# Eclectic-Sheep/sheeprl

Hardware: NVIDIA H100
Metric: Dreamer-V3 train-steps/sec (S, bs16 seq64 horizon15, 64x64x3 obs) (higher is better)
Workload: dtype f32

## Files before the change

sheeprl_b200/csrc/gemm_tc.cu:

```cuda
#include <cuda.h>
#include <cudaTypedefs.h>

#include <mutex>
#include <unordered_map>

#include "common.cuh"

namespace {

constexpr int BM = 128, BK = 32;
constexpr int NTHREADS = 384;
constexpr int NSPLIT_THREADS = 96;
constexpr int NCONS_WARPS = 8;
constexpr int PRODUCER_REGS = 56, CONSUMER_REGS = 224;
template <int PASSES, bool PRESPLIT> __host__ __device__ constexpr int b_buffers() { return PRESPLIT ? (PASSES == 3 ? 2 : 1) : 3; }
template <int BN, int PASSES, bool PRESPLIT> constexpr int stages_for() {
  return (227 * 1024 - 1024 - 256) / ((BM + b_buffers<PASSES, PRESPLIT>() * BN) * BK * (int)sizeof(float));
}

__device__ __forceinline__ uint32_t smem_u32(const void* p) { return (uint32_t)__cvta_generic_to_shared(p); }

__device__ __forceinline__ void mbar_init(uint64_t* bar, uint32_t count) {
  asm volatile("mbarrier.init.shared::cta.b64 [%0], %1;" ::"r"(smem_u32(bar)), "r"(count) : "memory");
}
__device__ __forceinline__ void mbar_expect_tx(uint64_t* bar, uint32_t bytes) {
  asm volatile("mbarrier.arrive.expect_tx.shared::cta.b64 _, [%0], %1;" ::"r"(smem_u32(bar)), "r"(bytes) : "memory");
}
__device__ __forceinline__ void mbar_arrive(uint64_t* bar) {
  asm volatile("mbarrier.arrive.shared::cta.b64 _, [%0];" ::"r"(smem_u32(bar)) : "memory");
}
__device__ __forceinline__ bool mbar_try_wait(uint64_t* bar, uint32_t parity) {
// ... 52 lines not shown
__device__ __forceinline__ void wgmma_tf32(float (&d)[64], const uint32_t (&a)[4], uint64_t desc_b, int scale_d) {
  asm volatile(
      "{\n\t.reg .pred p;\n\tsetp.ne.b32 p, %69, 0;\n\twgmma.mma_async.sync.aligned.m64n128k8.f32.tf32.tf32 {%0, %1, %2, %3, %4, %5, %6, %7, %8, %9, %10, %11, %12, %13, %14, %15, %16, %17, %18, %19, %20, %21, %22, %23, %24, %25, %26, %27, %28, %29, %30, %31, %32, %33, %34, %35, %36, %37, %38, %39, %40, %41, %42, %43, %44, %45, %46, %47, %48, %49, %50, %51, %52, %53, %54, %55, %56, %57, %58, %59, %60, %61, %62, %63}, {%64, %65, %66, %67}, %68, p, 1, 1;\n\t}"
      : "+f"(d[0]), "+f"(d[1]), "+f"(d[2]), "+f"(d[3]), "+f"(d[4]), "+f"(d[5]), "+f"(d[6]), "+f"(d[7]), "+f"(d[8]), "+f"(d[9]), "+f"(d[10]), "+f"(d[11]), "+f"(d[12]), "+f"(d[13]), "+f"(d[14]), "+f"(d[15]), "+f"(d[16]), "+f"(d[17]), "+f"(d[18]), "+f"(d[19]), "+f"(d[20]), "+f"(d[21]), "+f"(d[22]), "+f"(d[23]), "+f"(d[24]), "+f"(d[25]), "+f"(d[26]), "+f"(d[27]), "+f"(d[28]), "+f"(d[29]), "+f"(d[30]), "+f"(d[31]), "+f"(d[32]), "+f"(d[33]), "+f"(d[34]), "+f"(d[35]), "+f"(d[36]), "+f"(d[37]), "+f"(d[38]), "+f"(d[39]), "+f"(d[40]), "+f"(d[41]), "+f"(d[42]), "+f"(d[43]), "+f"(d[44]), "+f"(d[45]), "+f"(d[46]), "+f"(d[47]), "+f"(d[48]), "+f"(d[49]), "+f"(d[50]), "+f"(d[51]), "+f"(d[52]), "+f"(d[53]), "+f"(d[54]), "+f"(d[55]), "+f"(d[56]), "+f"(d[57]), "+f"(d[58]), "+f"(d[59]), "+f"(d[60]), "+f"(d[61]), "+f"(d[62]), "+f"(d[63])
      : "r"(a[0]), "r"(a[1]), "r"(a[2]), "r"(a[3]), "l"(desc_b), "r"(scale_d));
}
__device__ __forceinline__ void wgmma_fence() { asm volatile("wgmma.fence.sync.aligned;" ::: "memory"); }
__device__ __forceinline__ void wgmma_commit() { asm volatile("wgmma.commit_group.sync.aligned;" ::: "memory"); }
__device__ __forceinline__ void wgmma_wait_all() { asm volatile("wgmma.wait_group.sync.aligned 0;" ::: "memory"); }
template <int N>
__device__ __forceinline__ void fence_regs(float (&r)[N]) {
#pragma unroll
  for (int i = 0; i < N; ++i) asm volatile("" : "+f"(r[i])::"memory");
}
template <int N, int W>
__device__ __forceinline__ void fence_regs(uint32_t (&r)[N][W]) {
#pragma unroll
  for (int i = 0; i < N; ++i)
#pragma unroll
    for (int j = 0; j < W; ++j) asm volatile("" : "+r"(r[i][j])::"memory");
}

__device__ __forceinline__ uint64_t make_desc(uint32_t smem_addr) {
  uint64_t d = 0;
  d |= (uint64_t)((smem_addr & 0x3FFFF) >> 4);
  d |= (uint64_t)1 << 16;
  d |= (uint64_t)(1024 >> 4) << 32;
  d |= (uint64_t)1 << 62;
  return d;
}

__device__ __forceinline__ uint32_t kmajor_off(int r, int k) {
  return (uint32_t)(r * 128 + ((((k >> 2) ^ r) & 7) << 4) + (k & 3) * 4);
}
__device__ __forceinline__ uint32_t mnmajor_off(int r, int k) {
  return (uint32_t)((r >> 5) * 4096 + k * 128 + (((((r & 31) >> 2) ^ k) & 7) << 4) + (r & 3) * 4);
}

template <int BN, int PASSES, bool PRESPLIT>
struct Smem;
template <int BN, int PASSES>
struct Smem<BN, PASSES, false> {
  static constexpr int STAGES = stages_for<BN, PASSES, false>();
  float a[STAGES][BM * BK];
  float b[STAGES][BN * BK];
  float b_hi[STAGES][BN * BK];
  float b_lo[STAGES][BN * BK];
  uint64_t full[STAGES], split[STAGES], empty[STAGES];
};
template <int BN, int PASSES>
struct Smem<BN, PASSES, true> {
  static constexpr int STAGES = stages_for<BN, PASSES, true>();
  float a[STAGES][BM * BK];
  float b_hi[STAGES][BN * BK];
  float b_lo[PASSES == 3 ? STAGES : 1][PASSES == 3 ? BN * BK : 256];
  uint64_t full[STAGES], empty[STAGES];
};

constexpr int CH = 4;

constexpr int MODE_GEMM = 0, MODE_DOWN = 1, MODE_UP = 2;
constexpr int MODE_UP4 = 3;
constexpr int GROUP_M = 16;
struct TileGeo {
  int mode;
  int h, w, NB;
  int bw, bh, bn;
  int tiles_x, tiles_y;
  int chunks;
  int Cout;
  int ksplits;
  float* part;
  int mpad, ldw;
  int force_part;
  int passes;
  int a_mn, b_mn;
  int mtiles;
  int ntiles;
  int wg;
};

template <int BN, int PASSES, bool PRESPLIT>
__global__ void __launch_bounds__(NTHREADS, 1)
gemm_tc_kernel(const __grid_constant__ CUtensorMap mapA, const __grid_constant__ CUtensorMap mapB,
               const __grid_constant__ CUtensorMap mapBlo, float* __restrict__ C, const float* __restrict__ bias, int M,
               int N, int K, int ldc, int accumulate, const TileGeo geo) {
  using S = Smem<BN, PASSES, PRESPLIT>;
  constexpr int STAGES = S::STAGES;
  extern __shared__ __align__(1024) unsigned char smem_raw[];
  S& s = *reinterpret_cast<S*>(smem_raw + ((1024u - (smem_u32(smem_raw) & 1023u)) & 1023u));
  const int warp = threadIdx.x >> 5, lane = threadIdx.x & 31;
  const int mtiles = geo.mtiles * geo.ntiles, tstride = gridDim.y;
  auto tile_mn = [&](int id, int& tm, int& tn) {
    if (geo.ntiles == 1) { tm = id; tn = 0; return; }
    const int per = GROUP_M * geo.ntiles, grp = id / per, first = grp * GROUP_M;
    const int gsz = min(GROUP_M, geo.mtiles - first), r = id - grp * per;
    tn = r / gsz;
    tm = first + (r - tn * gsz);
  };
  int kb_base = 0, nkb = (K + BK - 1) / BK;
  if (geo.mode == MODE_GEMM && geo.ksplits > 1) {
    const int per = (nkb + geo.ksplits - 1) / geo.ksplits;
    kb_base = (int)blockIdx.z * per;
    nkb = min(per, nkb - kb_base);
  }
  const int py = (int)blockIdx.z >> 1, px = (int)blockIdx.z & 1;
  auto tile_origin = [&](int id, int& tx0, int& ty0, int& tn0) {
    tx0 = (id % geo.tiles_x) * geo.bw;
    ty0 = ((id / geo.tiles_x) % geo.tiles_y) * geo.bh;
    tn0 = (id / (geo.tiles_x * geo.tiles_y)) * geo.bn;
  };

  if (threadIdx.x == 0) {
    for (int i = 0; i < STAGES; ++i) {
      mbar_init(&s.full[i], 1);
      if constexpr (!PRESPLIT) mbar_init(&s.split[i], NSPLIT_THREADS / 32);
      mbar_init(&s.empty[i], NCONS_WARPS);
    }
    asm volatile("fence.mbarrier_init.release.cluster;" ::: "memory");
  }
  __syncthreads();

  if (warp < 4) {
    asm volatile("setmaxnreg.dec.sync.aligned.u32 %0;" ::"n"(PRODUCER_REGS));
    if (warp == 0) {
      const bool leader = elect_one();
      constexpr uint32_t STAGE_TX = (uint32_t)((BM + (PRESPLIT ? b_buffers<PASSES, true>() : 1) * BN) * BK * sizeof(float));
      auto load_b_kmajor = [&](int st, int k, int n) {
        if constexpr (PRESPLIT) {
          tma_load_2d(s.b_hi[st], &mapB, &s.full[st], k, n);
          if (PASSES == 3) tma_load_2d(s.b_lo[st], &mapBlo, &s.full[st], k, n);
        } else {
          tma_load_2d(s.b[st], &mapB, &s.full[st], k, n);
        }
      };
      int it = 0;
      for (int tile = blockIdx.y; tile < mtiles; tile += tstride) {
        int tm, tn;
        tile_mn(tile, tm, tn);
        const int m0 = tm * BM, n0 = tn * BN;
        int tx0 = 0, ty0 = 0, tn0 = 0;
        if (geo.mode != MODE_GEMM) tile_origin(tm, tx0, ty0, tn0);
        for (int kb = 0; kb < nkb; ++kb, ++it) {
          const int st = it % STAGES;
          if (it >= STAGES) mbar_wait(&s.empty[st], ((it / STAGES) - 1) & 1);
          if (leader) {
            mbar_expect_tx(&s.full[st], STAGE_TX);
            if (geo.mode == MODE_GEMM) {
              const int k0 = (kb_base + kb) * BK;
              if (geo.wg) {
                const int x0 = k0 % geo.w, y0 = (k0 / geo.w) % geo.h, i0 = k0 / (geo.w * geo.h);
                for (int j = 0; j < BM / 32; ++j) {
                  const int r0 = m0 + 32 * j, tap = r0 / geo.Cout, ch = r0 - tap * geo.Cout;
                  tma_load_4d(s.a[st] + j * 1024, &mapA, &s.full[st], ch, 2 * x0 - 1 + (tap & 3), 2 * y0 - 1 + (tap >> 2), i0);
                }
              } else if (!geo.a_mn) tma_load_2d(s.a[st], &mapA, &s.full[st], k0, m0);
              else
                for (int j = 0; j < BM / 32; ++j) tma_load_2d(s.a[st] + j * 1024, &mapA, &s.full[st], m0 + 32 * j, k0);
              if (PRESPLIT || !geo.b_mn) load_b_kmajor(st, k0, n0);
              else if constexpr (!PRESPLIT)
                for (int j = 0; j < BN / 32; ++j) tma_load_2d(s.b[st] + j * 1024, &mapB, &s.full[st], n0 + 32 * j, k0);
            } else {
              const int tap = kb / geo.chunks, ch = (kb - tap * geo.chunks) * BK;
              int x, y;
              if (geo.mode == MODE_DOWN)     { x = 2 * tx0 - 1 + (tap & 3); y = 2 * ty0 - 1 + (tap >> 2); }
              else if (geo.mode == MODE_UP4) { x = tx0 + (tap % 3) - 1;     y = ty0 + (tap / 3) - 1; }
              else                           { x = tx0 + px - (tap & 1);    y = ty0 + py - (tap >> 1); }
              tma_load_4d(s.a[st], &mapA, &s.full[st], ch, x, y, tn0);
              load_b_kmajor(st, kb * BK, n0 + (geo.mode == MODE_UP ? (int)blockIdx.z * geo.Cout : 0));
            }
          }
          __syncwarp();
        }
      }
    } else if constexpr (!PRESPLIT) {
      const int t = threadIdx.x - 32;
      int ntl = 0;
      for (int tile = blockIdx.y; tile < mtiles; tile += tstride) ++ntl;
      const int total_kb = ntl * nkb;
      const bool b_mn = geo.b_mn != 0;
      for (int kb = 0; kb < total_kb; ++kb) {
        const int st = kb % STAGES;
        mbar_wait(&s.full[st], (kb / STAGES) & 1);
        const char* raw = reinterpret_cast<const char*>(s.b[st]);
// ... 17 lines not shown
          h.x = __uint_as_float(__float_as_uint(v.x) & 0xffffe000u);
          h.y = __uint_as_float(__float_as_uint(v.y) & 0xffffe000u);
          h.z = __uint_as_float(__float_as_uint(v.z) & 0xffffe000u);
          h.w = __uint_as_float(__float_as_uint(v.w) & 0xffffe000u);
          const uint32_t o = kmajor_off(n, 4 * kc);
          *reinterpret_cast<float4*>(bh + o) = h;
          if (PASSES == 3) *reinterpret_cast<float4*>(bl + o) = make_float4(v.x - h.x, v.y - h.y, v.z - h.z, v.w - h.w);
        }
        asm volatile("fence.proxy.async.shared::cta;" ::: "memory");
        __syncwarp();
        if (lane == 0) mbar_arrive(&s.split[st]);
      }
    }
  } else {
    asm volatile("setmaxnreg.inc.sync.aligned.u32 %0;" ::"n"(CONSUMER_REGS));
    constexpr int NACC = BN / 2;
    const int cw = (warp >> 2) - 1, wq = warp & 3, g = lane >> 2, tq = lane & 3;
    const int r0 = cw * 64 + wq * 16 + g;
    const bool a_mn_tile = geo.a_mn != 0;
    const uint64_t dbh_base = make_desc(smem_u32(s.b_hi[0])), dbl_base = make_desc(smem_u32(s.b_lo[0]));
    constexpr uint64_t STAGE_STEP = (uint64_t)(BN * BK * sizeof(float)) >> 4;
    int it = 0;
    for (int tile = blockIdx.y; tile < mtiles; tile += tstride) {
      int tm, tn;
      tile_mn(tile, tm, tn);
      const int m0 = tm * BM, n0 = tn * BN;
      int tx0 = 0, ty0 = 0, tn0 = 0;
      if (geo.mode != MODE_GEMM) tile_origin(tm, tx0, ty0, tn0);
      float acc[NACC], cacc[NACC];
#pragma unroll
      for (int j = 0; j < NACC; ++j) { acc[j] = 0.f; cacc[j] = 0.f; }
      for (int kb = 0; kb < nkb; ++kb, ++it) {
        const int st = it % STAGES;
        const uint32_t ph = (it / STAGES) & 1;
        mbar_wait(&s.full[st], ph);
        if constexpr (!PRESPLIT) mbar_wait(&s.split[st], ph);
        const char* araw = reinterpret_cast<const char*>(s.a[st]);
        uint32_t ahi[4][4], alo[4][4];
#pragma unroll
        for (int ks = 0; ks < 4; ++ks)
#pragma unroll
          for (int e = 0; e < 4; ++e) {
            const int r = r0 + 8 * (e & 1), k = 8 * ks + tq + 4 * (e >> 1);
            const uint32_t x = *reinterpret_cast<const uint32_t*>(araw + (a_mn_tile ? mnmajor_off(r, k) : kmajor_off(r, k)));
            ahi[ks][e] = x & 0xffffe000u;
            if (PASSES == 3) alo[ks][e] = __float_as_uint(__uint_as_float(x) - __uint_as_float(x & 0xffffe000u));
          }
        const bool chunk_start = (kb % CH) == 0;
        const uint64_t dbh0 = dbh_base + (uint64_t)st * STAGE_STEP, dbl0 = dbl_base + (uint64_t)st * STAGE_STEP;
        fence_regs(cacc);
        fence_regs(ahi);
        if (PASSES == 3) fence_regs(alo);
        wgmma_fence();
#pragma unroll
        for (int ks = 0; ks < 4; ++ks) {
          const uint64_t ob = (uint64_t)ks * 2;
          const int keep = !(chunk_start && ks == 0);
          if (PASSES == 3) {
            wgmma_tf32(cacc, ahi[ks], dbl0 + ob, keep);
            wgmma_tf32(cacc, alo[ks], dbh0 + ob, 1);
            wgmma_tf32(cacc, ahi[ks], dbh0 + ob, 1);
          } else {
            wgmma_tf32(cacc, ahi[ks], dbh0 + ob, keep);
          }
        }
        wgmma_commit();
        wgmma_wait_all();
        fence_regs(cacc);
        fence_regs(ahi);
        if (PASSES == 3) fence_regs(alo);
        __syncwarp();
        if (lane == 0) mbar_arrive(&s.empty[st]);
        if ((kb % CH) == CH - 1 || kb == nkb - 1) {
#pragma unroll
          for (int j = 0; j < NACC; ++j) acc[j] += cacc[j];
        }
      }
#pragma unroll
      for (int hh = 0; hh < 2; ++hh) {
        const int r = r0 + 8 * hh;
        const int row = m0 + r;
        bool row_ok = row < M;
        size_t row_off = (size_t)row * ldc;
        int wi = 0, hi = 0, ni = 0;
        if (geo.mode != MODE_GEMM) {
          wi = r % geo.bw; hi = (r / geo.bw) % geo.bh; ni = r / (geo.bw * geo.bh);
          const int n = tn0 + ni, y = ty0 + hi, x = tx0 + wi;
          row_ok = n < geo.NB;
          if (geo.mode == MODE_DOWN) row_off = (((size_t)n * geo.h + y) * geo.w + x) * (size_t)ldc;
          else row_off = (((size_t)n * (2 * geo.h) + (2 * y + py)) * (2 * geo.w) + (2 * x + px)) * (size_t)ldc;
        }
        if (geo.mode == MODE_UP4) {
          if (!row_ok) continue;
          const size_t n = (size_t)(tn0 + ni);
          const int y = ty0 + hi, x = tx0 + wi;
#pragma unroll
          for (int j = 0; j < NACC / 4; ++j) {
            const int c = 8 * j + 2 * tq, p = c >> 5, ch = c & 31;
            float* dst = C + ((n * (2 * geo.h) + (2 * y + (p >> 1))) * (2 * geo.w) + (2 * x + (p & 1))) * (size_t)32 + ch;
            float2 o = make_float2(acc[4 * j + 2 * hh], acc[4 * j + 2 * hh + 1]);
            if (bias) { o.x += bias[ch]; o.y += bias[ch + 1]; }
            *reinterpret_cast<float2*>(dst) = o;
          }
          continue;
        }
        if (geo.mode == MODE_GEMM && (geo.ksplits > 1 || geo.force_part)) {
          float* prow = geo.part + ((size_t)blockIdx.z * geo.mpad + (size_t)row) * geo.ldw + n0;
#pragma unroll
          for (int j = 0; j < NACC / 4; ++j)
            *reinterpret_cast<float2*>(prow + 8 * j + 2 * tq) = make_float2(acc[4 * j + 2 * hh], acc[4 * j + 2 * hh + 1]);
          continue;
        }
        if (!row_ok) continue;
        float* crow = C + row_off;
#pragma unroll
        for (int j = 0; j < NACC / 4; ++j) {
          const int cb = n0 + 8 * j + 2 * tq;
          float v0 = acc[4 * j + 2 * hh], v1 = acc[4 * j + 2 * hh + 1];
          if (cb + 1 < N && ((reinterpret_cast<uintptr_t>(crow + cb) & 7) == 0)) {
            if (bias) { v0 += bias[cb]; v1 += bias[cb + 1]; }
            if (accumulate) { const float2 q = *reinterpret_cast<const float2*>(crow + cb); v0 += q.x; v1 += q.y; }
            *reinterpret_cast<float2*>(crow + cb) = make_float2(v0, v1);
          } else {
            if (cb < N) crow[cb] = v0 + (bias ? bias[cb] : 0.f) + (accumulate ? crow[cb] : 0.f);
            if (cb + 1 < N) crow[cb + 1] = v1 + (bias ? bias[cb + 1] : 0.f) + (accumulate ? crow[cb + 1] : 0.f);
          }
        }
      }
    }
  }
}

struct MapKey {
// ... 155 lines not shown
  store_split(P, L, idx, W[((long long)cs * Cb + cb) * 16 + tap]);
}
__global__ void conv_pack_up_kernel(const float* __restrict__ W, float* __restrict__ P, float* __restrict__ L, int Cs,
                                    int Cb) {
  const long long idx = (long long)blockIdx.x * blockDim.x + threadIdx.x;
  if (idx >= (long long)Cs * Cb * 16) return;
  const int cs = (int)(idx % Cs);
  const int t = (int)((idx / Cs) % 4);
  const int cb = (int)((idx / ((long long)Cs * 4)) % Cb);
  const int par = (int)(idx / ((long long)Cs * 4 * Cb));
  const int py = par >> 1, px = par & 1;
  const int ky = (1 - py) + 2 * (t >> 1), kx = (1 - px) + 2 * (t & 1);
  store_split(P, L, idx, W[((long long)cs * Cb + cb) * 16 + ky * 4 + kx]);
}

__global__ void conv_pack_up4_kernel(const float* __restrict__ W, float* __restrict__ P, float* __restrict__ L, int Cs,
                                     int Cb) {
  const long long idx = (long long)blockIdx.x * blockDim.x + threadIdx.x;
  if (idx >= 36LL * Cs * Cb) return;
  const int cs = (int)(idx % Cs);
  const int shift = (int)((idx / Cs) % 9);
  const int cb = (int)((idx / (9LL * Cs)) % Cb);
  const int par = (int)(idx / (9LL * Cs * Cb));
  const int py = par >> 1, px = par & 1, dy = shift / 3 - 1, dx = shift % 3 - 1;
  const int j = py - dy, i = px - dx;
  float v = 0.f;
  if (j >= 0 && j <= 1 && i >= 0 && i <= 1) v = W[((long long)cs * Cb + cb) * 16 + ((1 - py) + 2 * j) * 4 + (1 - px) + 2 * i];
  store_split(P, L, idx, v);
}
static bool conv_up_merged(int Cb) { return Cb == 32; }

int g_passes = 3;

struct SplitWs {
  float* part = nullptr;
  size_t floats = 0;
};
SplitWs g_split[16];
std::mutex g_split_mu;

int split_workspace(size_t need_floats, cudaStream_t st, float** part) {
  int dev = 0;
// ... 37 lines not shown
  if (n + 4 <= N && ((reinterpret_cast<uintptr_t>(c) & 15) == 0)) {
    float4 r = acc;
    if (bias) { r.x += bias[n]; r.y += bias[n + 1]; r.z += bias[n + 2]; r.w += bias[n + 3]; }
    if (accumulate) { const float4 q = *reinterpret_cast<const float4*>(c); r.x += q.x; r.y += q.y; r.z += q.z; r.w += q.w; }
    *reinterpret_cast<float4*>(c) = r;
  } else {
    for (int j = 0; j < 4 && n + j < N; ++j) {
      float r = o[j];
      if (bias) r += bias[n + j];
      if (accumulate) r += c[j];
      c[j] = r;
    }
  }
}

#define LAUNCH_GEMM_TC(BN_, PASSES_, PRE_, grid_, st_, ...)                                                          \
  do {                                                                                                               \
    static_assert(sizeof(Smem<BN_, PASSES_, PRE_>) + 1024 <= 227 * 1024, "operand stages exceed shared memory");     \
    const size_t smem__ = sizeof(Smem<BN_, PASSES_, PRE_>) + 1024;                                                   \
    RL_CUDA(cudaFuncSetAttribute(gemm_tc_kernel<BN_, PASSES_, PRE_>, cudaFuncAttributeMaxDynamicSharedMemorySize,     \
                                 (int)smem__));                                                                      \
    gemm_tc_kernel<BN_, PASSES_, PRE_><<<grid_, NTHREADS, smem__, st_>>>(__VA_ARGS__);                                \
  } while (0)
#define DISPATCH_GEMM_TC_PRE(BN_val, passes_val, PRE_, grid_, st_, ...)                        \
  do {                                                                                          \
    if ((BN_val) == 64) {                                                                       \
      if ((passes_val) == 3) LAUNCH_GEMM_TC(64, 3, PRE_, grid_, st_, __VA_ARGS__);              \
      else LAUNCH_GEMM_TC(64, 1, PRE_, grid_, st_, __VA_ARGS__);                                \
    } else {                                                                                    \
      if ((passes_val) == 3) LAUNCH_GEMM_TC(128, 3, PRE_, grid_, st_, __VA_ARGS__);             \
      else LAUNCH_GEMM_TC(128, 1, PRE_, grid_, st_, __VA_ARGS__);                               \
    }                                                                                           \
  } while (0)
#define DISPATCH_GEMM_TC(BN_val, passes_val, presplit_, grid_, st_, ma_, mb_, mb2_, ...)                    \
  do {                                                                                                       \
    if (presplit_) DISPATCH_GEMM_TC_PRE(BN_val, passes_val, true, grid_, st_, ma_, mb_, mb2_, __VA_ARGS__);  \
    else DISPATCH_GEMM_TC_PRE(BN_val, passes_val, false, grid_, st_, ma_, mb_, mb_, __VA_ARGS__);           \
  } while (0)

int launch_conv(int mode, const float* img, const float* Wp, const float* Wlo, float* out, const float* bias, int NB, int h,
                int w, int Cin, int Cout, cudaStream_t st) {
  TileGeo g = {};
  g.mode = mode; g.h = h; g.w = w; g.NB = NB; g.chunks = Cin / BK; g.Cout = Cout; g.ksplits = 1;
  g.passes = g_passes;
  RL_CHECK_ARG(conv_tile(h, w, NB, &g.bw, &g.bh, &g.bn), "image grid not tileable by 128 pixels");
  g.tiles_x = w / g.bw; g.tiles_y = h / g.bh;
  if (mode == MODE_UP && conv_up_merged(Cout)) mode = g.mode = MODE_UP4;
  const int taps = mode == MODE_DOWN ? 16 : (mode == MODE_UP4 ? 9 : 4);
  const int K = taps * Cin;
  CUtensorMap ma, mb;
  if (mode == MODE_DOWN) { if (int rc = get_map4(img, Cin, 2 * w, 2 * h, NB, g.bw, g.bh, g.bn, 2, &ma)) return rc; }
  else                   { if (int rc = get_map4(img, Cin, w, h, NB, g.bw, g.bh, g.bn, 1, &ma)) return rc; }
  const int BN = (mode == MODE_UP4) ? 128 : ((Cout <= 64) ? 64 : 128);
  const int brows = (mode == MODE_UP || mode == MODE_UP4) ? 4 * Cout : Cout;
  if (int rc = get_map(Wp, brows, K, K, BN, &mb)) return rc;
  CUtensorMap mb2 = mb;
  if (Wlo && g.passes == 3) { if (int rc = get_map(Wlo, brows, K, K, BN, &mb2)) return rc; }
  const int mtiles = g.tiles_x * g.tiles_y * (NB / g.bn);
  g.mtiles = mtiles;
  g.ntiles = (mode == MODE_UP4) ? 1 : (Cout + BN - 1) / BN;
  dim3 grid(1, 1, mode == MODE_UP ? 4 : 1);
  grid.y = persistent_grid_y(mtiles * g.ntiles, grid.z);
  const int M = NB * h * w;
  DISPATCH_GEMM_TC(BN, g.passes, Wlo != nullptr, grid, st, ma, mb, mb2, out, bias, M, Cout, K, Cout, 0, g);
  RL_CHECK_LAUNCH();
  return B200RL_OK;
}

}

extern "C" int b200rl_set_matmul_precision(int tf32_passes) {
  RL_CHECK_ARG(tf32_passes == 1 || tf32_passes == 3, "tf32_passes must be 3 (fp32-accurate 3xTF32) or 1 (single TF32 pass)");
  g_passes = tf32_passes;
  return B200RL_OK;
}
extern "C" int b200rl_get_matmul_precision(void) { return g_passes; }

extern "C" long long b200rl_conv_pack_floats(int mode_up, int Cs, int Cb) {
  return (mode_up && conv_up_merged(Cb) ? 36LL : 16LL) * Cs * Cb;
}
extern "C" int b200rl_conv_tc_supported(int mode_up, int NB, int h, int w, int Cs, int Cb) {
  int bw, bh, bn;
  if (!conv_tile(h, w, NB, &bw, &bh, &bn)) return 0;
  const int Cin = mode_up ? Cs : Cb, Cout = mode_up ? Cb : Cs;
  if (Cin % BK != 0 || Cout < 16 || Cout % 4 != 0) return 0;
  return 1;
}
namespace {
int conv_pack_impl(const float* W, float* P, float* L, int mode_up, int Cs, int Cb, cudaStream_t st) {
  const long long n = (long long)Cs * Cb * 16;
  if (mode_up && conv_up_merged(Cb)) conv_pack_up4_kernel<<<ceil_div(36LL * Cs * Cb, 256), 256, 0, st>>>(W, P, L, Cs, Cb);
  else if (mode_up) conv_pack_up_kernel<<<ceil_div(n, 256), 256, 0, st>>>(W, P, L, Cs, Cb);
  else conv_pack_down_kernel<<<ceil_div(n, 256), 256, 0, st>>>(W, P, L, Cs, Cb);
  RL_CHECK_LAUNCH();
  return B200RL_OK;
}
}
extern "C" int b200rl_conv_pack(const float* W, float* Wpacked, int mode_up, int Cs, int Cb, cudaStream_t st) {
  RL_CHECK_ARG(W && Wpacked, "null pointer");
  return conv_pack_impl(W, Wpacked, nullptr, mode_up, Cs, Cb, st);
}
extern "C" int b200rl_conv_pack_split(const float* W, float* Whi, float* Wlo, int mode_up, int Cs, int Cb, cudaStream_t st) {
  RL_CHECK_ARG(W && Whi && Wlo, "null pointer");
  return conv_pack_impl(W, Whi, Wlo, mode_up, Cs, Cb, st);
}
extern "C" int b200rl_conv_down_tc(const float* big, const float* Wpacked, float* small_, int NB, int h, int w, int Cs,
// ... 46 lines not shown
  if ((lda & 3) || (ldb & 3)) return 0;
  if ((reinterpret_cast<uintptr_t>(A) & 15) || (reinterpret_cast<uintptr_t>(B) & 15)) return 0;
  return 1;
}

namespace {
struct FusedTail { float* part; int ks, mpad, ldw; };

int gemm_tc_impl(const float* A, const float* B, const float* Blo, float* C, const float* bias, int M, int N, int K,
                 int lda, int ldb, int ldc, int transA, int transB, int accumulate, cudaStream_t st, FusedTail* fused) {
  RL_CHECK_ARG(A && B && (C || fused), "null pointer");
  RL_CHECK_ARG(b200rl_gemm_tc_supported(A, B, M, N, K, lda, ldb, transA, transB), "shape not eligible for the tensor-core path");
  RL_CHECK_ARG(!Blo || (transB && !(reinterpret_cast<uintptr_t>(Blo) & 15)), "pre-split B must be 16-byte aligned [N][K] planes");
  const int BN = (N <= 64) ? 64 : 128;
  CUtensorMap ma, mb, mb2;
  if (!transA) { if (int rc = get_map(A, M, K, lda, BM, &ma)) return rc; }
  else         { if (int rc = get_map(A, K, M, lda, 32, &ma)) return rc; }
  if (transB)  { if (int rc = get_map(B, N, K, ldb, BN, &mb)) return rc; }
  else         { if (int rc = get_map(B, K, N, ldb, 32, &mb)) return rc; }
  mb2 = mb;
  if (Blo && g_passes == 3) { if (int rc = get_map(Blo, N, K, ldb, BN, &mb2)) return rc; }
  dim3 grid((N + BN - 1) / BN, (M + BM - 1) / BM);
  TileGeo g = {};
  g.mode = MODE_GEMM;
  g.a_mn = transA ? 1 : 0;
  g.b_mn = transB ? 0 : 1;
  g.ksplits = 1;
  g.passes = g_passes;
  const int tiles = grid.x * grid.y, nkb = (K + BK - 1) / BK;
  if (tiles < 2 * kNumSMs && nkb >= 8) {
    int best = 1;
    float best_t = 1e30f;
    const int max_sp = nkb / 4 < 32 ? nkb / 4 : 32;
    for (int sp = 1; sp <= (max_sp < 1 ? 1 : max_sp); ++sp) {
      const int per = (nkb + sp - 1) / sp, real = (nkb + per - 1) / per;
      const int waves = (tiles * real + kNumSMs - 1) / kNumSMs;
      const float t = waves * (per * 0.8f + 4.0f) + (real > 1 ? 3.0f + 0.3f * real : 0.0f);
      if (t < best_t - 1e-3f) { best_t = t; best = real; }
    }
    g.ksplits = best;
  }
  if (g.ksplits > 1 || fused) {
    grid.z = g.ksplits;
    g.mpad = (int)grid.y * BM;
    g.ldw = (int)grid.x * BN;
    if (int rc = split_workspace((size_t)g.ksplits * g.mpad * g.ldw, st, &g.part)) return rc;
    if (fused) { g.force_part = 1; *fused = FusedTail{g.part, g.ksplits, g.mpad, g.ldw}; }
  }
  g.mtiles = (int)grid.y;
  g.ntiles = (int)grid.x;
  grid.x = 1;
  grid.y = persistent_grid_y(g.mtiles * g.ntiles, grid.z);
  DISPATCH_GEMM_TC(BN, g.passes, Blo != nullptr, grid, st, ma, mb, mb2, C, bias, M, N, K, ldc, accumulate, g);
  RL_CHECK_LAUNCH();
  if (g.ksplits > 1 && !fused) {
    splitk_reduce_kernel<<<ceil_div((long long)M * ((N + 3) / 4), 256), 256, 0, st>>>(g.part, C, bias, M, N, ldc, g.ksplits, g.mpad,
                                                                                      g.ldw, accumulate);
    RL_CHECK_LAUNCH();
  }
  return B200RL_OK;
}

template <int NV>
__global__ void __launch_bounds__(256)
splitk_ln_kernel(const float* __restrict__ part, int ks, int mpad, int ldw, int M, int N, const float* __restrict__ gamma,
                 const float* __restrict__ beta, float eps, int act, float* __restrict__ pre, long long ldpre,
                 float* __restrict__ ln_out, long long ldln, int mode, const float* __restrict__ h_prev, long long ldh,
                 float* __restrict__ h_out, long long ldho, float* __restrict__ h_out2, long long ldho2) {
// ... 154 lines not shown
  return (bw * bh * bn == 32) && (NB % bn == 0);
}

extern "C" int b200rl_conv_wgrad_mn(const float* small_, const float* big, float* G, int NB, int h, int w, int Cs, int Cb,
                                    cudaStream_t st) {
  RL_CHECK_ARG(small_ && big && G, "null pointer");
  RL_CHECK_ARG(b200rl_conv_wgrad_mn_supported(NB, h, w, Cs, Cb), "shape not eligible for the in-place wgrad path");
  const int P = NB * h * w, M = 16 * Cb, N = Cs;
  TileGeo g = {};
  g.mode = MODE_GEMM; g.a_mn = 1; g.b_mn = 1; g.wg = 1; g.passes = g_passes;
  g.h = h; g.w = w; g.NB = NB; g.Cout = Cb;
  g.bw = w < 32 ? w : 32; g.bh = (32 / g.bw) < h ? (32 / g.bw) : h; g.bn = 32 / (g.bw * g.bh);
  CUtensorMap ma, mb;
  if (int rc = get_map4(big, Cb, 2 * w, 2 * h, NB, g.bw, g.bh, g.bn, 2, &ma)) return rc;
  if (int rc = get_map(small_, P, Cs, Cs, 32, &mb)) return rc;
  const int BN = (N <= 64) ? 64 : 128;
  dim3 grid((N + BN - 1) / BN, M / BM);
  const int tiles = grid.x * grid.y, nkb = P / BK;
  int sp = (2 * kNumSMs + tiles - 1) / tiles;
  if (sp > nkb / 8) sp = nkb / 8;
  if (sp < 1) sp = 1;
  const int per = (nkb + sp - 1) / sp;
  g.ksplits = (nkb + per - 1) / per;
  grid.z = g.ksplits;
  g.mtiles = (int)grid.y;
  g.ntiles = (int)grid.x;
  if (g.ksplits > 1) {
    g.mpad = (int)grid.y * BM;
    g.ldw = (int)grid.x * BN;
    if (int rc = split_workspace((size_t)g.ksplits * g.mpad * g.ldw, st, &g.part)) return rc;
  }
  grid.x = 1;
  grid.y = (unsigned)(g.mtiles * g.ntiles);
  DISPATCH_GEMM_TC(BN, g.passes, false, grid, st, ma, mb, mb, G, nullptr, M, N, P, N, 0, g);
  RL_CHECK_LAUNCH();
  if (g.ksplits > 1) {
    splitk_reduce_kernel<<<ceil_div((long long)M * ((N + 3) / 4), 256), 256, 0, st>>>(g.part, G, nullptr, M, N, N, g.ksplits, g.mpad,
                                                                                      g.ldw, 0);
    RL_CHECK_LAUNCH();
  }
  return B200RL_OK;
}
```

Baseline: 62.21.

## Add 256x64 conv GEMM tiles and split merged upconv by output row parity

Adds a BM template parameter so the TMA warp-specialized GEMM can use 256x64 tiles, with each consumer warpgroup covering two 64-row subtiles and the producer loading two 128-pixel boxes per stage. Conv and wgrad paths with BN=64 now use the taller tile, which reuses each B stage across twice as many rows. The merged 4-parity transposed conv (9 taps, BN=128) becomes a 6-tap, 2-launch-slice variant split by row parity, with BN=64, so fewer zero-padded taps are multiplied. Costs include fewer pipeline stages from the larger A tile, higher register pressure from doubled accumulators, and partial-tile handling through a 'live' flag.

```diff
diff --git a/sheeprl_b200/csrc/gemm_tc.cu b/sheeprl_b200/csrc/gemm_tc.cu
--- a/sheeprl_b200/csrc/gemm_tc.cu
+++ b/sheeprl_b200/csrc/gemm_tc.cu
@@ -8,13 +8,14 @@
 
 namespace {
 
-constexpr int BM = 128, BK = 32;
+constexpr int BK = 32;
+constexpr int BOX_M = 128;
 constexpr int NTHREADS = 384;
 constexpr int NSPLIT_THREADS = 96;
 constexpr int NCONS_WARPS = 8;
 constexpr int PRODUCER_REGS = 56, CONSUMER_REGS = 224;
 template <int PASSES, bool PRESPLIT> __host__ __device__ constexpr int b_buffers() { return PRESPLIT ? (PASSES == 3 ? 2 : 1) : 3; }
-template <int BN, int PASSES, bool PRESPLIT> constexpr int stages_for() {
+template <int BN, int BM, int PASSES, bool PRESPLIT> constexpr int stages_for() {
   return (227 * 1024 - 1024 - 256) / ((BM + b_buffers<PASSES, PRESPLIT>() * BN) * BK * (int)sizeof(float));
 }
 
@@ -97,11 +98,18 @@
   for (int i = 0; i < N; ++i) asm volatile("" : "+f"(r[i])::"memory");
 }
 template <int N, int W>
-__device__ __forceinline__ void fence_regs(uint32_t (&r)[N][W]) {
-#pragma unroll
-  for (int i = 0; i < N; ++i)
-#pragma unroll
-    for (int j = 0; j < W; ++j) asm volatile("" : "+r"(r[i][j])::"memory");
+__device__ __forceinline__ void fence_regs(float (&r)[N][W]) {
+#pragma unroll
+  for (int i = 0; i < N; ++i) fence_regs(r[i]);
+}
+template <int S, int N, int W>
+__device__ __forceinline__ void fence_regs(uint32_t (&r)[S][N][W]) {
+#pragma unroll
+  for (int s = 0; s < S; ++s)
+#pragma unroll
+    for (int i = 0; i < N; ++i)
+#pragma unroll
+      for (int j = 0; j < W; ++j) asm volatile("" : "+r"(r[s][i][j])::"memory");
 }
 
 __device__ __forceinline__ uint64_t make_desc(uint32_t smem_addr) {
@@ -120,20 +128,20 @@
   return (uint32_t)((r >> 5) * 4096 + k * 128 + (((((r & 31) >> 2) ^ k) & 7) << 4) + (r & 3) * 4);
 }
 
-template <int BN, int PASSES, bool PRESPLIT>
+template <int BN, int BM, int PASSES, bool PRESPLIT>
 struct Smem;
-template <int BN, int PASSES>
-struct Smem<BN, PASSES, false> {
-  static constexpr int STAGES = stages_for<BN, PASSES, false>();
+template <int BN, int BM, int PASSES>
+struct Smem<BN, BM, PASSES, false> {
+  static constexpr int STAGES = stages_for<BN, BM, PASSES, false>();
   float a[STAGES][BM * BK];
   float b[STAGES][BN * BK];
   float b_hi[STAGES][BN * BK];
   float b_lo[STAGES][BN * BK];
   uint64_t full[STAGES], split[STAGES], empty[STAGES];
 };
-template <int BN, int PASSES>
-struct Smem<BN, PASSES, true> {
-  static constexpr int STAGES = stages_for<BN, PASSES, true>();
+template <int BN, int BM, int PASSES>
+struct Smem<BN, BM, PASSES, true> {
+  static constexpr int STAGES = stages_for<BN, BM, PASSES, true>();
   float a[STAGES][BM * BK];
   float b_hi[STAGES][BN * BK];
   float b_lo[PASSES == 3 ? STAGES : 1][PASSES == 3 ? BN * BK : 256];
@@ -143,13 +151,14 @@
 constexpr int CH = 4;
 
 constexpr int MODE_GEMM = 0, MODE_DOWN = 1, MODE_UP = 2;
-constexpr int MODE_UP4 = 3;
+constexpr int MODE_UP2 = 3;
 constexpr int GROUP_M = 16;
 struct TileGeo {
   int mode;
   int h, w, NB;
   int bw, bh, bn;
   int tiles_x, tiles_y;
+  int boxes;
   int chunks;
   int Cout;
   int ksplits;
@@ -163,12 +172,14 @@
   int wg;
 };
 
-template <int BN, int PASSES, bool PRESPLIT>
+template <int BN, int BM, int PASSES, bool PRESPLIT>
 __global__ void __launch_bounds__(NTHREADS, 1)
 gemm_tc_kernel(const __grid_constant__ CUtensorMap mapA, const __grid_constant__ CUtensorMap mapB,
                const __grid_constant__ CUtensorMap mapBlo, float* __restrict__ C, const float* __restrict__ bias, int M,
                int N, int K, int ldc, int accumulate, const TileGeo geo) {
-  using S = Smem<BN, PASSES, PRESPLIT>;
+  static_assert(BM == BOX_M || (BM == 2 * BOX_M && BN == 64), "tile shapes: 128 x 64, 128 x 128, 256 x 64");
+  constexpr int MBOX = BM / BOX_M;
+  using S = Smem<BN, BM, PASSES, PRESPLIT>;
   constexpr int STAGES = S::STAGES;
   extern __shared__ __align__(1024) unsigned char smem_raw[];
   S& s = *reinterpret_cast<S*>(smem_raw + ((1024u - (smem_u32(smem_raw) & 1023u)) & 1023u));
@@ -187,7 +198,7 @@
     kb_base = (int)blockIdx.z * per;
     nkb = min(per, nkb - kb_base);
   }
-  const int py = (int)blockIdx.z >> 1, px = (int)blockIdx.z & 1;
+  const int py = geo.mode == MODE_UP2 ? (int)blockIdx.z : (int)blockIdx.z >> 1, px = (int)blockIdx.z & 1;
   auto tile_origin = [&](int id, int& tx0, int& ty0, int& tn0) {
     tx0 = (id % geo.tiles_x) * geo.bw;
     ty0 = ((id / geo.tiles_x) % geo.tiles_y) * geo.bh;
@@ -208,7 +219,7 @@
     asm volatile("setmaxnreg.dec.sync.aligned.u32 %0;" ::"n"(PRODUCER_REGS));
     if (warp == 0) {
       const bool leader = elect_one();
-      constexpr uint32_t STAGE_TX = (uint32_t)((BM + (PRESPLIT ? b_buffers<PASSES, true>() : 1) * BN) * BK * sizeof(float));
+      constexpr int B_TX_ROWS = (PRESPLIT ? b_buffers<PASSES, true>() : 1) * BN;
       auto load_b_kmajor = [&](int st, int k, int n) {
         if constexpr (PRESPLIT) {
           tma_load_2d(s.b_hi[st], &mapB, &s.full[st], k, n);
@@ -222,13 +233,17 @@
         int tm, tn;
         tile_mn(tile, tm, tn);
         const int m0 = tm * BM, n0 = tn * BN;
-        int tx0 = 0, ty0 = 0, tn0 = 0;
-        if (geo.mode != MODE_GEMM) tile_origin(tm, tx0, ty0, tn0);
+        int nbox = MBOX, tx0[MBOX] = {}, ty0[MBOX] = {}, tn0[MBOX] = {};
+        if (geo.mode != MODE_GEMM) {
+          if constexpr (MBOX > 1) nbox = min(MBOX, geo.boxes - tm * MBOX);
+          for (int b = 0; b < nbox; ++b) tile_origin(tm * MBOX + b, tx0[b], ty0[b], tn0[b]);
+        }
+        const uint32_t stage_tx = (uint32_t)((nbox * BOX_M + B_TX_ROWS) * BK * sizeof(float));
         for (int kb = 0; kb < nkb; ++kb, ++it) {
           const int st = it % STAGES;
           if (it >= STAGES) mbar_wait(&s.empty[st], ((it / STAGES) - 1) & 1);
           if (leader) {
-            mbar_expect_tx(&s.full[st], STAGE_TX);
+            mbar_expect_tx(&s.full[st], stage_tx);
             if (geo.mode == MODE_GEMM) {
               const int k0 = (kb_base + kb) * BK;
               if (geo.wg) {
@@ -237,20 +252,24 @@
                   const int r0 = m0 + 32 * j, tap = r0 / geo.Cout, ch = r0 - tap * geo.Cout;
                   tma_load_4d(s.a[st] + j * 1024, &mapA, &s.full[st], ch, 2 * x0 - 1 + (tap & 3), 2 * y0 - 1 + (tap >> 2), i0);
                 }
-              } else if (!geo.a_mn) tma_load_2d(s.a[st], &mapA, &s.full[st], k0, m0);
-              else
+              } else if (!geo.a_mn) {
+                for (int b = 0; b < MBOX; ++b) tma_load_2d(s.a[st] + b * BOX_M * BK, &mapA, &s.full[st], k0, m0 + b * BOX_M);
+              } else
                 for (int j = 0; j < BM / 32; ++j) tma_load_2d(s.a[st] + j * 1024, &mapA, &s.full[st], m0 + 32 * j, k0);
               if (PRESPLIT || !geo.b_mn) load_b_kmajor(st, k0, n0);
               else if constexpr (!PRESPLIT)
                 for (int j = 0; j < BN / 32; ++j) tma_load_2d(s.b[st] + j * 1024, &mapB, &s.full[st], n0 + 32 * j, k0);
             } else {
               const int tap = kb / geo.chunks, ch = (kb - tap * geo.chunks) * BK;
-              int x, y;
-              if (geo.mode == MODE_DOWN)     { x = 2 * tx0 - 1 + (tap & 3); y = 2 * ty0 - 1 + (tap >> 2); }
-              else if (geo.mode == MODE_UP4) { x = tx0 + (tap % 3) - 1;     y = ty0 + (tap / 3) - 1; }
-              else                           { x = tx0 + px - (tap & 1);    y = ty0 + py - (tap >> 1); }
-              tma_load_4d(s.a[st], &mapA, &s.full[st], ch, x, y, tn0);
-              load_b_kmajor(st, kb * BK, n0 + (geo.mode == MODE_UP ? (int)blockIdx.z * geo.Cout : 0));
+              for (int b = 0; b < nbox; ++b) {
+                int x, y;
+                if (geo.mode == MODE_DOWN)     { x = 2 * tx0[b] - 1 + (tap & 3); y = 2 * ty0[b] - 1 + (tap >> 2); }
+                else if (geo.mode == MODE_UP2) { x = tx0[b] + (tap % 3) - 1;     y = ty0[b] + py - 1 + tap / 3; }
+                else                           { x = tx0[b] + px - (tap & 1);    y = ty0[b] + py - (tap >> 1); }
+                tma_load_4d(s.a[st] + b * BOX_M * BK, &mapA, &s.full[st], ch, x, y, tn0[b]);
+              }
+              load_b_kmajor(st, kb * BK, n0 + (geo.mode == MODE_UP ? (int)blockIdx.z * geo.Cout
+                                                : geo.mode == MODE_UP2 ? py * 2 * geo.Cout : 0));
             }
           }
           __syncwarp();
@@ -298,9 +317,9 @@
     }
   } else {
     asm volatile("setmaxnreg.inc.sync.aligned.u32 %0;" ::"n"(CONSUMER_REGS));
-    constexpr int NACC = BN / 2;
+    constexpr int NACC = BN / 2, MSUB = BM / 128;
     const int cw = (warp >> 2) - 1, wq = warp & 3, g = lane >> 2, tq = lane & 3;
-    const int r0 = cw * 64 + wq * 16 + g;
+    const int r0 = cw * (BM / 2) + wq * 16 + g;
     const bool a_mn_tile = geo.a_mn != 0;
     const uint64_t dbh_base = make_desc(smem_u32(s.b_hi[0])), dbl_base = make_desc(smem_u32(s.b_lo[0]));
     constexpr uint64_t STAGE_STEP = (uint64_t)(BN * BK * sizeof(float)) >> 4;
@@ -309,80 +328,93 @@
       int tm, tn;
       tile_mn(tile, tm, tn);
       const int m0 = tm * BM, n0 = tn * BN;
-      int tx0 = 0, ty0 = 0, tn0 = 0;
-      if (geo.mode != MODE_GEMM) tile_origin(tm, tx0, ty0, tn0);
-      float acc[NACC], cacc[NACC];
-#pragma unroll
-      for (int j = 0; j < NACC; ++j) { acc[j] = 0.f; cacc[j] = 0.f; }
+      const bool live = MBOX == 1 || geo.mode == MODE_GEMM || (m0 + cw * (BM / 2)) / BOX_M < geo.boxes;
+      float acc[MSUB][NACC], cacc[MSUB][NACC];
+#pragma unroll
+      for (int sb = 0; sb < MSUB; ++sb)
+#pragma unroll
+        for (int j = 0; j < NACC; ++j) { acc[sb][j] = 0.f; cacc[sb][j] = 0.f; }
       for (int kb = 0; kb < nkb; ++kb, ++it) {
         const int st = it % STAGES;
         const uint32_t ph = (it / STAGES) & 1;
         mbar_wait(&s.full[st], ph);
         if constexpr (!PRESPLIT) mbar_wait(&s.split[st], ph);
-        const char* araw = reinterpret_cast<const char*>(s.a[st]);
-        uint32_t ahi[4][4], alo[4][4];
-#pragma unroll
-        for (int ks = 0; ks < 4; ++ks)
-#pragma unroll
-          for (int e = 0; e < 4; ++e) {
-            const int r = r0 + 8 * (e & 1), k = 8 * ks + tq + 4 * (e >> 1);
-            const uint32_t x = *reinterpret_cast<const uint32_t*>(araw + (a_mn_tile ? mnmajor_off(r, k) : kmajor_off(r, k)));
-            ahi[ks][e] = x & 0xffffe000u;
-            if (PASSES == 3) alo[ks][e] = __float_as_uint(__uint_as_float(x) - __uint_as_float(x & 0xffffe000u));
-          }
-        const bool chunk_start = (kb % CH) == 0;
-        const uint64_t dbh0 = dbh_base + (uint64_t)st * STAGE_STEP, dbl0 = dbl_base + (uint64_t)st * STAGE_STEP;
-        fence_regs(cacc);
-        fence_regs(ahi);
-        if (PASSES == 3) fence_regs(alo);
-        wgmma_fence();
-#pragma unroll
-        for (int ks = 0; ks < 4; ++ks) {
-          const uint64_t ob = (uint64_t)ks * 2;
-          const int keep = !(chunk_start && ks == 0);
-          if (PASSES == 3) {
-            wgmma_tf32(cacc, ahi[ks], dbl0 + ob, keep);
-            wgmma_tf32(cacc, alo[ks], dbh0 + ob, 1);
-            wgmma_tf32(cacc, ahi[ks], dbh0 + ob, 1);
-          } else {
-            wgmma_tf32(cacc, ahi[ks], dbh0 + ob, keep);
-          }
+        if (live) {
+          const char* araw = reinterpret_cast<const char*>(s.a[st]);
+          uint32_t ahi[MSUB][4][4], alo[MSUB][4][4];
+#pragma unroll
+          for (int sb = 0; sb < MSUB; ++sb)
+#pragma unroll
+            for (int ks = 0; ks < 4; ++ks)
+#pragma unroll
+              for (int e = 0; e < 4; ++e) {
+                const int r = r0 + 64 * sb + 8 * (e & 1), k = 8 * ks + tq + 4 * (e >> 1);
+                const uint32_t x = *reinterpret_cast<const uint32_t*>(araw + (a_mn_tile ? mnmajor_off(r, k) : kmajor_off(r, k)));
+                ahi[sb][ks][e] = x & 0xffffe000u;
+                if (PASSES == 3) alo[sb][ks][e] = __float_as_uint(__uint_as_float(x) - __uint_as_float(x & 0xffffe000u));
+              }
+          const bool chunk_start = (kb % CH) == 0;
+          const uint64_t dbh0 = dbh_base + (uint64_t)st * STAGE_STEP, dbl0 = dbl_base + (uint64_t)st * STAGE_STEP;
+          fence_regs(cacc);
+          fence_regs(ahi);
+          if (PASSES == 3) fence_regs(alo);
+          wgmma_fence();
+#pragma unroll
+          for (int sb = 0; sb < MSUB; ++sb)
+#pragma unroll
+            for (int ks = 0; ks < 4; ++ks) {
+              const uint64_t ob = (uint64_t)ks * 2;
+              const int keep = !(chunk_start && ks == 0);
+              if (PASSES == 3) {
+                wgmma_tf32(cacc[sb], ahi[sb][ks], dbl0 + ob, keep);
+                wgmma_tf32(cacc[sb], alo[sb][ks], dbh0 + ob, 1);
+                wgmma_tf32(cacc[sb], ahi[sb][ks], dbh0 + ob, 1);
+              } else {
+                wgmma_tf32(cacc[sb], ahi[sb][ks], dbh0 + ob, keep);
+              }
+            }
+          wgmma_commit();
+          wgmma_wait_all();
+          fence_regs(cacc);
+          fence_regs(ahi);
+          if (PASSES == 3) fence_regs(alo);
         }
-        wgmma_commit();
-        wgmma_wait_all();
-        fence_regs(cacc);
-        fence_regs(ahi);
-        if (PASSES == 3) fence_regs(alo);
         __syncwarp();
         if (lane == 0) mbar_arrive(&s.empty[st]);
         if ((kb % CH) == CH - 1 || kb == nkb - 1) {
 #pragma unroll
-          for (int j = 0; j < NACC; ++j) acc[j] += cacc[j];
+          for (int sb = 0; sb < MSUB; ++sb)
+#pragma unroll
+            for (int j = 0; j < NACC; ++j) acc[sb][j] += cacc[sb][j];
         }
       }
+      if (!live) continue;
+#pragma unroll
+      for (int sb = 0; sb < MSUB; ++sb)
 #pragma unroll
       for (int hh = 0; hh < 2; ++hh) {
-        const int r = r0 + 8 * hh;
+        const float* a = acc[sb];
+        const int r = r0 + 64 * sb + 8 * hh;
         const int row = m0 + r;
         bool row_ok = row < M;
         size_t row_off = (size_t)row * ldc;
-        int wi = 0, hi = 0, ni = 0;
+        int n = 0, y = 0, x = 0;
         if (geo.mode != MODE_GEMM) {
-          wi = r % geo.bw; hi = (r / geo.bw) % geo.bh; ni = r / (geo.bw * geo.bh);
-          const int n = tn0 + ni, y = ty0 + hi, x = tx0 + wi;
+          int tx0, ty0, tn0;
+          tile_origin(row / BOX_M, tx0, ty0, tn0);
+          const int rb = row % BOX_M;
+          x = tx0 + rb % geo.bw; y = ty0 + (rb / geo.bw) % geo.bh; n = tn0 + rb / (geo.bw * geo.bh);
           row_ok = n < geo.NB;
           if (geo.mode == MODE_DOWN) row_off = (((size_t)n * geo.h + y) * geo.w + x) * (size_t)ldc;
           else row_off = (((size_t)n * (2 * geo.h) + (2 * y + py)) * (2 * geo.w) + (2 * x + px)) * (size_t)ldc;
         }
-        if (geo.mode == MODE_UP4) {
+        if (geo.mode == MODE_UP2) {
           if (!row_ok) continue;
-          const size_t n = (size_t)(tn0 + ni);
-          const int y = ty0 + hi, x = tx0 + wi;
 #pragma unroll
           for (int j = 0; j < NACC / 4; ++j) {
-            const int c = 8 * j + 2 * tq, p = c >> 5, ch = c & 31;
-            float* dst = C + ((n * (2 * geo.h) + (2 * y + (p >> 1))) * (2 * geo.w) + (2 * x + (p & 1))) * (size_t)32 + ch;
-            float2 o = make_float2(acc[4 * j + 2 * hh], acc[4 * j + 2 * hh + 1]);
+            const int c = 8 * j + 2 * tq, q = c >> 5, ch = c & 31;
+            float* dst = C + (((size_t)n * (2 * geo.h) + (2 * y + py)) * (2 * geo.w) + (2 * x + q)) * (size_t)32 + ch;
+            float2 o = make_float2(a[4 * j + 2 * hh], a[4 * j + 2 * hh + 1]);
             if (bias) { o.x += bias[ch]; o.y += bias[ch + 1]; }
             *reinterpret_cast<float2*>(dst) = o;
           }
@@ -392,7 +424,7 @@
           float* prow = geo.part + ((size_t)blockIdx.z * geo.mpad + (size_t)row) * geo.ldw + n0;
 #pragma unroll
           for (int j = 0; j < NACC / 4; ++j)
-            *reinterpret_cast<float2*>(prow + 8 * j + 2 * tq) = make_float2(acc[4 * j + 2 * hh], acc[4 * j + 2 * hh + 1]);
+            *reinterpret_cast<float2*>(prow + 8 * j + 2 * tq) = make_float2(a[4 * j + 2 * hh], a[4 * j + 2 * hh + 1]);
           continue;
         }
         if (!row_ok) continue;
@@ -400,7 +432,7 @@
 #pragma unroll
         for (int j = 0; j < NACC / 4; ++j) {
           const int cb = n0 + 8 * j + 2 * tq;
-          float v0 = acc[4 * j + 2 * hh], v1 = acc[4 * j + 2 * hh + 1];
+          float v0 = a[4 * j + 2 * hh], v1 = a[4 * j + 2 * hh + 1];
           if (cb + 1 < N && ((reinterpret_cast<uintptr_t>(crow + cb) & 7) == 0)) {
             if (bias) { v0 += bias[cb]; v1 += bias[cb + 1]; }
             if (accumulate) { const float2 q = *reinterpret_cast<const float2*>(crow + cb); v0 += q.x; v1 += q.y; }
@@ -586,18 +618,20 @@
   store_split(P, L, idx, W[((long long)cs * Cb + cb) * 16 + ky * 4 + kx]);
 }
 
-__global__ void conv_pack_up4_kernel(const float* __restrict__ W, float* __restrict__ P, float* __restrict__ L, int Cs,
+__global__ void conv_pack_up2_kernel(const float* __restrict__ W, float* __restrict__ P, float* __restrict__ L, int Cs,
                                      int Cb) {
   const long long idx = (long long)blockIdx.x * blockDim.x + threadIdx.x;
   if (idx >= 36LL * Cs * Cb) return;
-  const int cs = (int)(idx % Cs);
-  const int shift = (int)((idx / Cs) % 9);
-  const int cb = (int)((idx / (9LL * Cs)) % Cb);
-  const int par = (int)(idx / (9LL * Cs * Cb));
-  const int py = par >> 1, px = par & 1, dy = shift / 3 - 1, dx = shift % 3 - 1;
-  const int j = py - dy, i = px - dx;
   float v = 0.f;
-  if (j >= 0 && j <= 1 && i >= 0 && i <= 1) v = W[((long long)cs * Cb + cb) * 16 + ((1 - py) + 2 * j) * 4 + (1 - px) + 2 * i];
+  if (idx < 24LL * Cs * Cb) {
+    const int cs = (int)(idx % Cs);
+    const int shift = (int)((idx / Cs) % 6);
+    const int cb = (int)((idx / (6LL * Cs)) % Cb);
+    const int par = (int)(idx / (6LL * Cs * Cb));
+    const int py = par >> 1, px = par & 1, dy = py - 1 + shift / 3, dx = shift % 3 - 1;
+    const int j = py - dy, i = px - dx;
+    if (i >= 0 && i <= 1) v = W[((long long)cs * Cb + cb) * 16 + ((1 - py) + 2 * j) * 4 + (1 - px) + 2 * i];
+  }
   store_split(P, L, idx, v);
 }
 static bool conv_up_merged(int Cb) { return Cb == 32; }
@@ -665,28 +699,29 @@
   }
 }
 
-#define LAUNCH_GEMM_TC(BN_, PASSES_, PRE_, grid_, st_, ...)                                                          \
+#define LAUNCH_GEMM_TC(BN_, BM_, PASSES_, PRE_, grid_, st_, ...)                                                      \
   do {                                                                                                               \
-    static_assert(sizeof(Smem<BN_, PASSES_, PRE_>) + 1024 <= 227 * 1024, "operand stages exceed shared memory");     \
-    const size_t smem__ = sizeof(Smem<BN_, PASSES_, PRE_>) + 1024;                                                   \
-    RL_CUDA(cudaFuncSetAttribute(gemm_tc_kernel<BN_, PASSES_, PRE_>, cudaFuncAttributeMaxDynamicSharedMemorySize,     \
+    static_assert(sizeof(Smem<BN_, BM_, PASSES_, PRE_>) + 1024 <= 227 * 1024, "operand stages exceed shared memory"); \
+    const size_t smem__ = sizeof(Smem<BN_, BM_, PASSES_, PRE_>) + 1024;                                              \
+    RL_CUDA(cudaFuncSetAttribute(gemm_tc_kernel<BN_, BM_, PASSES_, PRE_>, cudaFuncAttributeMaxDynamicSharedMemorySize, \
                                  (int)smem__));                                                                      \
-    gemm_tc_kernel<BN_, PASSES_, PRE_><<<grid_, NTHREADS, smem__, st_>>>(__VA_ARGS__);                                \
+    gemm_tc_kernel<BN_, BM_, PASSES_, PRE_><<<grid_, NTHREADS, smem__, st_>>>(__VA_ARGS__);                           \
   } while (0)
-#define DISPATCH_GEMM_TC_PRE(BN_val, passes_val, PRE_, grid_, st_, ...)                        \
-  do {                                                                                          \
-    if ((BN_val) == 64) {                                                                       \
-      if ((passes_val) == 3) LAUNCH_GEMM_TC(64, 3, PRE_, grid_, st_, __VA_ARGS__);              \
-      else LAUNCH_GEMM_TC(64, 1, PRE_, grid_, st_, __VA_ARGS__);                                \
-    } else {                                                                                    \
-      if ((passes_val) == 3) LAUNCH_GEMM_TC(128, 3, PRE_, grid_, st_, __VA_ARGS__);             \
-      else LAUNCH_GEMM_TC(128, 1, PRE_, grid_, st_, __VA_ARGS__);                               \
-    }                                                                                           \
+#define DISPATCH_GEMM_TC_PASSES(BN_, BM_, passes_val, PRE_, grid_, st_, ...)               \
+  do {                                                                                      \
+    if ((passes_val) == 3) LAUNCH_GEMM_TC(BN_, BM_, 3, PRE_, grid_, st_, __VA_ARGS__);      \
+    else LAUNCH_GEMM_TC(BN_, BM_, 1, PRE_, grid_, st_, __VA_ARGS__);                        \
   } while (0)
-#define DISPATCH_GEMM_TC(BN_val, passes_val, presplit_, grid_, st_, ma_, mb_, mb2_, ...)                    \
-  do {                                                                                                       \
-    if (presplit_) DISPATCH_GEMM_TC_PRE(BN_val, passes_val, true, grid_, st_, ma_, mb_, mb2_, __VA_ARGS__);  \
-    else DISPATCH_GEMM_TC_PRE(BN_val, passes_val, false, grid_, st_, ma_, mb_, mb_, __VA_ARGS__);           \
+#define DISPATCH_GEMM_TC_PRE(BN_val, BM_val, passes_val, PRE_, grid_, st_, ...)                          \
+  do {                                                                                                    \
+    if ((BN_val) == 128) DISPATCH_GEMM_TC_PASSES(128, 128, passes_val, PRE_, grid_, st_, __VA_ARGS__);    \
+    else if ((BM_val) == 256) DISPATCH_GEMM_TC_PASSES(64, 256, passes_val, PRE_, grid_, st_, __VA_ARGS__); \
+    else DISPATCH_GEMM_TC_PASSES(64, 128, passes_val, PRE_, grid_, st_, __VA_ARGS__);                     \
+  } while (0)
+#define DISPATCH_GEMM_TC(BN_val, BM_val, passes_val, presplit_, grid_, st_, ma_, mb_, mb2_, ...)                    \
+  do {                                                                                                               \
+    if (presplit_) DISPATCH_GEMM_TC_PRE(BN_val, BM_val, passes_val, true, grid_, st_, ma_, mb_, mb2_, __VA_ARGS__);  \
+    else DISPATCH_GEMM_TC_PRE(BN_val, BM_val, passes_val, false, grid_, st_, ma_, mb_, mb_, __VA_ARGS__);           \
   } while (0)
 
 int launch_conv(int mode, const float* img, const float* Wp, const float* Wlo, float* out, const float* bias, int NB, int h,
@@ -696,24 +731,25 @@
   g.passes = g_passes;
   RL_CHECK_ARG(conv_tile(h, w, NB, &g.bw, &g.bh, &g.bn), "image grid not tileable by 128 pixels");
   g.tiles_x = w / g.bw; g.tiles_y = h / g.bh;
-  if (mode == MODE_UP && conv_up_merged(Cout)) mode = g.mode = MODE_UP4;
-  const int taps = mode == MODE_DOWN ? 16 : (mode == MODE_UP4 ? 9 : 4);
+  if (mode == MODE_UP && conv_up_merged(Cout)) mode = g.mode = MODE_UP2;
+  const int taps = mode == MODE_DOWN ? 16 : (mode == MODE_UP2 ? 6 : 4);
   const int K = taps * Cin;
   CUtensorMap ma, mb;
   if (mode == MODE_DOWN) { if (int rc = get_map4(img, Cin, 2 * w, 2 * h, NB, g.bw, g.bh, g.bn, 2, &ma)) return rc; }
   else                   { if (int rc = get_map4(img, Cin, w, h, NB, g.bw, g.bh, g.bn, 1, &ma)) return rc; }
-  const int BN = (mode == MODE_UP4) ? 128 : ((Cout <= 64) ? 64 : 128);
-  const int brows = (mode == MODE_UP || mode == MODE_UP4) ? 4 * Cout : Cout;
+  const int BN = (mode == MODE_UP2 || Cout <= 64) ? 64 : 128;
+  const int BM = BN == 64 ? 256 : 128;
+  const int brows = (mode == MODE_UP || mode == MODE_UP2) ? 4 * Cout : Cout;
   if (int rc = get_map(Wp, brows, K, K, BN, &mb)) return rc;
   CUtensorMap mb2 = mb;
   if (Wlo && g.passes == 3) { if (int rc = get_map(Wlo, brows, K, K, BN, &mb2)) return rc; }
-  const int mtiles = g.tiles_x * g.tiles_y * (NB / g.bn);
-  g.mtiles = mtiles;
-  g.ntiles = (mode == MODE_UP4) ? 1 : (Cout + BN - 1) / BN;
-  dim3 grid(1, 1, mode == MODE_UP ? 4 : 1);
-  grid.y = persistent_grid_y(mtiles * g.ntiles, grid.z);
+  g.boxes = g.tiles_x * g.tiles_y * (NB / g.bn);
+  g.mtiles = ceil_div(g.boxes, BM / BOX_M);
+  g.ntiles = (mode == MODE_UP2) ? 1 : (Cout + BN - 1) / BN;
+  dim3 grid(1, 1, mode == MODE_UP ? 4 : (mode == MODE_UP2 ? 2 : 1));
+  grid.y = persistent_grid_y(g.mtiles * g.ntiles, grid.z);
   const int M = NB * h * w;
-  DISPATCH_GEMM_TC(BN, g.passes, Wlo != nullptr, grid, st, ma, mb, mb2, out, bias, M, Cout, K, Cout, 0, g);
+  DISPATCH_GEMM_TC(BN, BM, g.passes, Wlo != nullptr, grid, st, ma, mb, mb2, out, bias, M, Cout, K, Cout, 0, g);
   RL_CHECK_LAUNCH();
   return B200RL_OK;
 }
@@ -740,7 +776,7 @@
 namespace {
 int conv_pack_impl(const float* W, float* P, float* L, int mode_up, int Cs, int Cb, cudaStream_t st) {
   const long long n = (long long)Cs * Cb * 16;
-  if (mode_up && conv_up_merged(Cb)) conv_pack_up4_kernel<<<ceil_div(36LL * Cs * Cb, 256), 256, 0, st>>>(W, P, L, Cs, Cb);
+  if (mode_up && conv_up_merged(Cb)) conv_pack_up2_kernel<<<ceil_div(36LL * Cs * Cb, 256), 256, 0, st>>>(W, P, L, Cs, Cb);
   else if (mode_up) conv_pack_up_kernel<<<ceil_div(n, 256), 256, 0, st>>>(W, P, L, Cs, Cb);
   else conv_pack_down_kernel<<<ceil_div(n, 256), 256, 0, st>>>(W, P, L, Cs, Cb);
   RL_CHECK_LAUNCH();
@@ -817,13 +853,13 @@
   RL_CHECK_ARG(!Blo || (transB && !(reinterpret_cast<uintptr_t>(Blo) & 15)), "pre-split B must be 16-byte aligned [N][K] planes");
   const int BN = (N <= 64) ? 64 : 128;
   CUtensorMap ma, mb, mb2;
-  if (!transA) { if (int rc = get_map(A, M, K, lda, BM, &ma)) return rc; }
+  if (!transA) { if (int rc = get_map(A, M, K, lda, BOX_M, &ma)) return rc; }
   else         { if (int rc = get_map(A, K, M, lda, 32, &ma)) return rc; }
   if (transB)  { if (int rc = get_map(B, N, K, ldb, BN, &mb)) return rc; }
   else         { if (int rc = get_map(B, K, N, ldb, 32, &mb)) return rc; }
   mb2 = mb;
   if (Blo && g_passes == 3) { if (int rc = get_map(Blo, N, K, ldb, BN, &mb2)) return rc; }
-  dim3 grid((N + BN - 1) / BN, (M + BM - 1) / BM);
+  dim3 grid((N + BN - 1) / BN, (M + BOX_M - 1) / BOX_M);
   TileGeo g = {};
   g.mode = MODE_GEMM;
   g.a_mn = transA ? 1 : 0;
@@ -845,7 +881,7 @@
   }
   if (g.ksplits > 1 || fused) {
     grid.z = g.ksplits;
-    g.mpad = (int)grid.y * BM;
+    g.mpad = (int)grid.y * BOX_M;
     g.ldw = (int)grid.x * BN;
     if (int rc = split_workspace((size_t)g.ksplits * g.mpad * g.ldw, st, &g.part)) return rc;
     if (fused) { g.force_part = 1; *fused = FusedTail{g.part, g.ksplits, g.mpad, g.ldw}; }
@@ -854,7 +890,7 @@
   g.ntiles = (int)grid.x;
   grid.x = 1;
   grid.y = persistent_grid_y(g.mtiles * g.ntiles, grid.z);
-  DISPATCH_GEMM_TC(BN, g.passes, Blo != nullptr, grid, st, ma, mb, mb2, C, bias, M, N, K, ldc, accumulate, g);
+  DISPATCH_GEMM_TC(BN, BOX_M, g.passes, Blo != nullptr, grid, st, ma, mb, mb2, C, bias, M, N, K, ldc, accumulate, g);
   RL_CHECK_LAUNCH();
   if (g.ksplits > 1 && !fused) {
     splitk_reduce_kernel<<<ceil_div((long long)M * ((N + 3) / 4), 256), 256, 0, st>>>(g.part, C, bias, M, N, ldc, g.ksplits, g.mpad,
@@ -1039,25 +1075,23 @@
   CUtensorMap ma, mb;
   if (int rc = get_map4(big, Cb, 2 * w, 2 * h, NB, g.bw, g.bh, g.bn, 2, &ma)) return rc;
   if (int rc = get_map(small_, P, Cs, Cs, 32, &mb)) return rc;
-  const int BN = (N <= 64) ? 64 : 128;
-  dim3 grid((N + BN - 1) / BN, M / BM);
-  const int tiles = grid.x * grid.y, nkb = P / BK;
-  int sp = (2 * kNumSMs + tiles - 1) / tiles;
+  const int BN = (N <= 64) ? 64 : 128, BM = BN == 64 ? 256 : 128;
+  const int tiles128 = ((N + BN - 1) / BN) * (M / BOX_M), nkb = P / BK;
+  int sp = (2 * kNumSMs + tiles128 - 1) / tiles128;
   if (sp > nkb / 8) sp = nkb / 8;
   if (sp < 1) sp = 1;
   const int per = (nkb + sp - 1) / sp;
   g.ksplits = (nkb + per - 1) / per;
-  grid.z = g.ksplits;
-  g.mtiles = (int)grid.y;
-  g.ntiles = (int)grid.x;
+  dim3 grid(1, 1, g.ksplits);
+  g.mtiles = M / BM;
+  g.ntiles = (N + BN - 1) / BN;
   if (g.ksplits > 1) {
-    g.mpad = (int)grid.y * BM;
-    g.ldw = (int)grid.x * BN;
+    g.mpad = M;
+    g.ldw = g.ntiles * BN;
     if (int rc = split_workspace((size_t)g.ksplits * g.mpad * g.ldw, st, &g.part)) return rc;
   }
-  grid.x = 1;
   grid.y = (unsigned)(g.mtiles * g.ntiles);
-  DISPATCH_GEMM_TC(BN, g.passes, false, grid, st, ma, mb, mb, G, nullptr, M, N, P, N, 0, g);
+  DISPATCH_GEMM_TC(BN, BM, g.passes, false, grid, st, ma, mb, mb, G, nullptr, M, N, P, N, 0, g);
   RL_CHECK_LAUNCH();
   if (g.ksplits > 1) {
     splitk_reduce_kernel<<<ceil_div((long long)M * ((N + 3) / 4), 256), 256, 0, st>>>(g.part, G, nullptr, M, N, N, g.ksplits, g.mpad,
```

After: 62.88, median of 6. 1.1% higher.
